# anyboby/Constrained-Model-Based-Policy-Optimization

Measured on AMD Instinct MI355X. Metric: imagined env-steps/sec (ensemble rollout) + CPO update ms, higher is better.
Workload: dtype f32; 1 GPU; AntSafe-v2 imagined rollout: E=7 x (37->512->512->60) swish ensemble, 5 elites, 3+3 critics 128x128, tanh policy 128x128, B=100000 branches/GPU, maxroll 35 (34 steps), fixed-horizon mode, reset->sample*->finish_all_paths->get(); rollout_mode=schedule, branches_per_gpu=100000, branches_total=100000, horizon=34, task=AntSafe-v2

## Files before the change

constrained-model-based-policy-optimization_amd/csrc/ens_h3.hip:

```cpp
#include "common.h"
#include "ens_mlp_internal.h"
#include "f16_split.h"

#include <stdlib.h>

#include <type_traits>

namespace {

constexpr int kThreadsH = 512;
constexpr int kWavesH = 8;
constexpr int HIDH = 512;

template <int RT>
struct Geo {
  static constexpr int ROWS = 32 * RT;
  static constexpr int NTC = 8 / RT;
  static constexpr int CK = 32 * NTC;
  static constexpr int NCH = HIDH / CK;
  static constexpr int SLC = CK / 16;
  static constexpr int CSTR = CK + 8;
  static constexpr int TPR = kThreadsH / ROWS;
  static constexpr int KPT = 64 / TPR;
  static constexpr int DA = RT == 4 ? 2 : 4;
  static constexpr int CBUF_BYTES = 2 * ROWS * CSTR * 2;
  static constexpr bool W0_LDS = RT == 4;
};

constexpr int PBUF_BYTES = kWavesH * 2 * 16 * 64 * 4;
constexpr int SWS = 65;
constexpr int STG_BYTES = 32 * SWS * 4;
__host__ __device__ constexpr int ximg_bytes(int S0, int RT) { return 2 * 32 * RT * (16 * S0 + 8) * 2; }
__host__ __device__ constexpr int w0buf_bytes(int S0, int RT) { return RT == 4 ? 2 * S0 * 2 * 1024 : 0; }
__host__ __device__ constexpr int off_const(int S0, int RT) {
  const int cb = RT == 4 ? Geo<4>::CBUF_BYTES : (RT == 2 ? Geo<2>::CBUF_BYTES : Geo<1>::CBUF_BYTES);
  const int a = 2 * cb + ximg_bytes(S0, RT) + 2 * w0buf_bytes(S0, RT), b = 2 * PBUF_BYTES + 2 * STG_BYTES;
  return ((a > b ? a : b) + 15) / 16 * 16;
}
constexpr int CONST_FLOATS = 2 * HIDH + 2 * 128 + 6 * 128 + 2 * 64;
// ... 33 lines not shown
  __shared__ float red[3][kThreadsH];
  red[0][tid] = wmax; red[1][tid] = l1; red[2][tid] = bmax;
  __syncthreads();
  for (int st = kThreadsH / 2; st > 0; st >>= 1) {
    if (tid < st)
      for (int q = 0; q < 3; ++q) red[q][tid] = fmaxf(red[q][tid], red[q][tid + st]);
    __syncthreads();
  }
  if (tid == 0) {
    float *o = stats + (size_t)e * NSTAT + 4 * l;
    o[0] = pow2_lift(red[0][0]); o[1] = red[1][0]; o[2] = red[2][0]; o[3] = red[0][0];
  }
}

__global__ void h3_pack_kernel(const float *src, size_t src_stride, int kg, int src_tiles, f16x8 *dst, size_t dst_stride,
                               int n_tiles, int slabs, int members, const float *stats, int layer, int perm) {
  const long idx = (long)blockIdx.x * blockDim.x + threadIdx.x;
  const long per = (long)n_tiles * slabs * 64;
  if (idx >= per * members) return;
  const int e = (int)(idx / per);
  const int rem = (int)(idx - (long)e * per);
  const int lane = rem & 63, s = (rem >> 6) % slabs, tile = (rem >> 6) / slabs;
  const int r = lane & 31, h = lane >> 5;
  const float scale = stats[(size_t)e * NSTAT + 4 * layer];
  const float *sp = src + (size_t)e * src_stride;
  f16x8 p1, p2;
#pragma unroll
  for (int j = 0; j < 8; ++j) {
    int k = 16 * s + 8 * h + j;
    if (perm) {
      const int i = 8 * (s & 1) + j;
      k = 32 * (s >> 1) + (i & 3) + 8 * (i >> 2) + 4 * h;
    }
    float v = 0.0f;
    if (tile < src_tiles && (k >> 3) < kg) v = sp[(((size_t)tile * kg + (k >> 3)) * 64 + ((k >> 2) & 1) * 32 + r) * 4 + (k & 3)];
    _Float16 q1, q2;
    split_h(v * scale, q1, q2);
    p1[j] = q1; p2[j] = q2;
  }
  f16x8 *d = dst + (size_t)e * dst_stride + ((size_t)tile * slabs + s) * 2 * 64 + lane;
  d[0] = p1; d[64] = p2;
}

template <int I, int N, class F>
__device__ __forceinline__ void static_for(F &&f) {
  if constexpr (I < N) {
    f(std::integral_constant<int, I>{});
    static_for<I + 1, N>(f);
  }
}

#ifdef H3_FULL_BARRIERS
#define H3_BARRIER() __syncthreads()
#else
#define H3_BARRIER() asm volatile("s_waitcnt lgkmcnt(0)\n\ts_barrier" ::: "memory")
#endif

#ifndef H3_EPI_FUSE
#define H3_EPI_FUSE 1
#endif
#ifndef IN_SCALE_RCP
#define IN_SCALE_RCP 1
#endif
#ifndef H3_PEEL_LAST
#define H3_PEEL_LAST 1
#endif
#ifndef H3_STORE8
#define H3_STORE8 1
#endif
#ifndef H3_TAIL_RING
#define H3_TAIL_RING 0
#endif

struct H3Args {
  MlpKernelArgs m;
  const f16x8 *w0, *w1, *w2;
  size_t w0_stride, w1_stride, w2_stride;
  const float *stats;
  int item0;
};

template <int S0, int OTP, int RT>
__global__ __launch_bounds__(kThreadsH, 2) void ens_h3_kernel(const H3Args a) {
  using G = Geo<RT>;
  constexpr int ROWSH = G::ROWS, NTC = G::NTC, CK = G::CK, NCH = G::NCH, SLC = G::SLC, CSTR = G::CSTR, TPR = G::TPR,
                KPT = G::KPT, DA = G::DA, CBUF_BYTES = G::CBUF_BYTES;
  constexpr int XSTR = 16 * S0 + 8;
  constexpr int NPASS = OTP / 2;
  constexpr int NUNIT = RT * NPASS;
  constexpr int O_PAD = 32 * OTP;
  constexpr int W0P = NTC * S0 * 2;
  const MlpKernelArgs &p = a.m;
  extern __shared__ f32x4 smem4[];
  char *smem = reinterpret_cast<char *>(smem4);
  _Float16 *cbuf = reinterpret_cast<_Float16 *>(smem);
  _Float16 *ximg = reinterpret_cast<_Float16 *>(smem + 2 * CBUF_BYTES);
  f16x8 *w0buf = reinterpret_cast<f16x8 *>(smem + 2 * CBUF_BYTES + ximg_bytes(S0, RT));
  f32x4 *pbuf = reinterpret_cast<f32x4 *>(smem);
  float *stg = reinterpret_cast<float *>(smem + 2 * PBUF_BYTES);
  float *cst = reinterpret_cast<float *>(smem + off_const(S0, RT));
  float *bias0 = cst, *bias1 = cst + HIDH, *hc_a = cst + 2 * HIDH, *hc_c = hc_a + 128;
// ... 154 lines not shown
      const f16x8 *wa = G::W0_LDS ? w0buf + ((size_t)(cc & 1) * W0P + (size_t)l0_tn * S0 * 2 + 2 * s) * 64 + lane
                                  : w0e + (((size_t)(cc < NCH ? cc : NCH - 1) * NTC + l0_tn) * S0 * 2 + 2 * s) * 64 + lane;
      o.a1 = wa[0]; o.a2 = wa[64];
      o.b1 = *reinterpret_cast<const f16x8 *>(xb0 + 16 * s);
      o.b2 = *reinterpret_cast<const f16x8 *>(xb0 + (size_t)ROWSH * XSTR + 16 * s);
    };
    auto l0_store = [&](const Epi4 &s, int cc, int q) {
      _Float16 *c1 = cbuf + (size_t)(cc & 1) * (CBUF_BYTES / 2) + (size_t)(32 * l0_bt + r) * CSTR + 32 * l0_tn + 4 * hh + 8 * q;
      *reinterpret_cast<uint2 *>(c1) = make_uint2(s.q1[0], s.q1[1]);
      *reinterpret_cast<uint2 *>(c1 + (size_t)ROWSH * CSTR) = make_uint2(s.q2[0], s.q2[1]);
    };
    auto l0_bias = [&](int cc, int q) {
      return *reinterpret_cast<const f32x4 *>(bias0 + cc * CK + 32 * l0_tn + 8 * q + 4 * hh);
    };

    f32x16 acc[2][RT];
#pragma unroll
    for (int t = 0; t < 2; ++t)
#pragma unroll
      for (int bt = 0; bt < RT; ++bt)
#pragma unroll
        for (int i = 0; i < 16; ++i) acc[t][bt][i] = 0.0f;
    const f16x8 *w1a = a.w1 + (size_t)e * a.w1_stride + (size_t)(2 * wave) * 32 * 128 + lane;
    f16x8 A[DA][2][2];
    f16x8 Bt[3][2];
    auto load_a = [&](f16x8 (&x)[2][2], int s) {
#pragma unroll
      for (int t = 0; t < 2; ++t) {
        const f16x8 *q = w1a + ((size_t)t * 32 + s) * 128;
        x[t][0] = q[0]; x[t][1] = q[64];
      }
    };
    auto read_bt = [&](f16x8 (&x)[2], const _Float16 *img, int bt, int sl) {
      const _Float16 *q = img + (size_t)(32 * bt + r) * CSTR + 16 * sl + 8 * hh;
      x[0] = *reinterpret_cast<const f16x8 *>(q);
      x[1] = *reinterpret_cast<const f16x8 *>(q + (size_t)ROWSH * CSTR);
    };
#pragma unroll
    for (int s = 0; s < DA - 1; ++s) load_a(A[s], s);
    {
      f32x16 d;
#pragma unroll
      for (int i = 0; i < 16; ++i) d[i] = 0.0f;
#pragma unroll
      for (int s = 0; s < S0; ++s) {
        L0Ops o;
        l0_read(o, 0, s);
        mm3(d, o.a1, o.a2, o.b1, o.b2);
      }
#pragma unroll
      for (int q = 0; q < 4; ++q) {
        Epi4 es;
        const f32x4 bv = l0_bias(0, q);
        epi_all<false, true, H3_EPI_FUSE>(es, d, q, inv0_l, bv, t1_l);
        l0_store(es, 0, q);
      }
    }
    H3_BARRIER();
    H3_STAMP(2);

    auto step = [&](auto LASTC, const int c) {
      constexpr bool LAST = decltype(LASTC)::value;
      f16x8 wst;
      const bool stage_w0 = c + 2 < NCH;
      const int cw = stage_w0 ? c + 2 : NCH - 1;
      const _Float16 *img = cbuf + (size_t)(c & 1) * (CBUF_BYTES / 2);
      f32x16 d;
#pragma unroll
      for (int i = 0; i < 16; ++i) d[i] = 0.0f;
      L0Ops l0;
      Epi4 es;
      f32x4 bv = {0.0f, 0.0f, 0.0f, 0.0f};
      read_bt(Bt[0], img, 0, 0);
      read_bt(Bt[1], img, 1 % RT, 1 / RT);
      if constexpr (!LAST) l0_read(l0, c + 1, 0);
#pragma unroll
      for (int slot = 0; slot < 8; ++slot) {
        if (!LAST && slot >= 4) bv = l0_bias(c + 1, slot - 4);
        if constexpr (G::W0_LDS && !LAST) {
          if (slot == 4) wst = w0e[((size_t)cw * W0P + wave) * 64 + lane];
          if (slot == 5 && W0P > kWavesH) {
            if (stage_w0) w0buf[((size_t)(c & 1) * W0P + wave) * 64 + lane] = wst;
            wst = w0e[((size_t)cw * W0P + (wave + kWavesH < W0P ? wave + kWavesH : wave)) * 64 + lane];
          }
        }
#pragma unroll
        for (int i = 0; i < 12; ++i) {
          const int pos = 2 * slot + i / 6;
          const int sl = pos / RT, bt = pos % RT;
          const int t = (i / 3) % 2, term = i % 3;
          if (i % 6 == 0) {
#ifndef H3_DIAG_NOA
            if (bt == 0) {
              const int sn = c * SLC + sl + DA - 1;
              load_a(A[(sl + DA - 1) % DA], sn < 32 ? sn : 31);
            }
#endif
#ifndef H3_DIAG_NOBT
            if (pos + 2 < 16) read_bt(Bt[(pos + 2) % 3], img, (pos + 2) % RT, (pos + 2) / RT);
#endif
            if (i == 0) __builtin_amdgcn_sched_barrier(0);
          }
          f16x8(&Ac)[2][2] = A[sl % DA];
          f32x16 &ac = acc[t][bt];
          const f16x8 &b1 = Bt[pos % 3][0], &b2 = Bt[pos % 3][1];
          if (term == 0) ac = __builtin_amdgcn_mfma_f32_32x32x16_f16(Ac[t][1], b1, ac, 0, 0, 0);
          else if (term == 1) ac = __builtin_amdgcn_mfma_f32_32x32x16_f16(Ac[t][0], b2, ac, 0, 0, 0);
          else ac = __builtin_amdgcn_mfma_f32_32x32x16_f16(Ac[t][0], b1, ac, 0, 0, 0);
#ifndef H3_DIAG_NOL0
          if (!LAST && slot < S0 && i == 5) {
            mm3(d, l0.a1, l0.a2, l0.b1, l0.b2);
            if (slot + 1 < S0) l0_read(l0, c + 1, slot + 1);
          }
#endif
#ifdef H3_DIAG_NOEPI_LOOP
          if (false) {
#else
          if (!LAST && slot >= 4) {
#endif
            const int q = slot - 4;
            if (i == 0) epi_stage<0, true, true, H3_EPI_FUSE>(es, d, q, inv0_l, bv, t1_l);
            if (i == 1) epi_stage<1, true, true, H3_EPI_FUSE>(es, d, q, inv0_l, bv, t1_l);
            if (i == 2) epi_stage<2, true, true, H3_EPI_FUSE>(es, d, q, inv0_l, bv, t1_l);
            if (i == 3) epi_stage<3, true, true, H3_EPI_FUSE>(es, d, q, inv0_l, bv, t1_l);
            if (i == 4) epi_stage<4, true, true, H3_EPI_FUSE>(es, d, q, inv0_l, bv, t1_l);
            if (i == 5) epi_stage<5, true, true, H3_EPI_FUSE>(es, d, q, inv0_l, bv, t1_l);
            if (i == 6) epi_stage<6, true, true, H3_EPI_FUSE>(es, d, q, inv0_l, bv, t1_l);
            if (i == 7) epi_stage<7, true, true, H3_EPI_FUSE>(es, d, q, inv0_l, bv, t1_l);
            if (i == 8) epi_stage<8, true, true, H3_EPI_FUSE>(es, d, q, inv0_l, bv, t1_l);
            if (i == 9) epi_stage<9, true, true, H3_EPI_FUSE>(es, d, q, inv0_l, bv, t1_l);
            if (i == 10) l0_store(es, c + 1, q);
          }
          __builtin_amdgcn_sched_barrier(0);
        }
      }
      H3_STAMP(4);
      if constexpr (G::W0_LDS && !LAST) {
        if (stage_w0) {
          const int j = W0P > kWavesH ? wave + kWavesH : wave;
          if (j < W0P) w0buf[((size_t)(c & 1) * W0P + j) * 64 + lane] = wst;
        }
      }
      H3_BARRIER();
      H3_STAMP(5);
    };
#if H3_PEEL_LAST
#pragma unroll 1
    for (int c = 0; c < NCH - 1; ++c) step(std::false_type{}, c);
    step(std::true_type{}, NCH - 1);
#else
#pragma unroll 1
    for (int c = 0; c < NCH; ++c) step(std::false_type{}, c);
#endif

    fetch_x(tid);
    fetch_bias(item + gridDim.x, tid);
    H3_STAMP(6);
#ifdef H3_DIAG_NOTAIL
    {
      float keep = 0.0f;
#pragma unroll
      for (int t = 0; t < 2; ++t)
#pragma unroll
        for (int bt = 0; bt < RT; ++bt)
#pragma unroll
          for (int i = 0; i < 16; ++i) keep += acc[t][bt][i];
      if (keep == 123.456f) p.out0[0] = keep;
    }
    H3_BARRIER();
    continue;
#endif

    const f16x8 *w2w = a.w2 + (size_t)e * a.w2_stride + lane + (size_t)(4 * wave) * 128;
    auto reduce_unit = [&](int u) {
      const int rt = u / NPASS, pass = u % NPASS;
      const int tt = wave >> 2, q = wave & 3;
      const f32x4 *pp = pbuf + ((size_t)(u & 1) * 64 + (size_t)tt * 4 + q) * 64 + lane;
      f32x4 v = pp[0];
#pragma unroll
      for (int wv = 1; wv < kWavesH; ++wv) v += pp[(size_t)wv * 8 * 64];
      const int nl = 32 * tt + 8 * q + 4 * hh, n = 64 * pass + nl;
      const f32x4 ha = *reinterpret_cast<const f32x4 *>(hc_a + n), hc = *reinterpret_cast<const f32x4 *>(hc_c + n);
      const float inv2_l = r_inv2[32 * rt + r];
      float *sg = stg + (size_t)(u & 1) * 32 * SWS + r * SWS + nl;
#pragma unroll
      for (int s = 0; s < 4; ++s) {
        float y = ha[s] * (v[s] * inv2_l) + hc[s];
        if (n + s >= out) y = __expf(y);
// ... 19 lines not shown
        return;
      }
      const int n = 64 * pass + lane;
#pragma unroll
      for (int j = 0; j < 4; ++j) {
        const int rl = wave + kWavesH * j;
        const int rr = rowidx[32 * rt + rl];
        const float y = stg[(size_t)(u & 1) * 32 * SWS + rl * SWS + lane];
        if (rr >= 0 && n < 2 * out) {
          const size_t obase = ((size_t)e * p.ld_rows + rr) * out;
          if (n < out) p.out0[obase + n] = y;
          else p.out1[obase + (n - out)] = y;
        }
      }
    };
    if constexpr (NPASS == 1 && !H3_TAIL_RING) {
      f16x8 w2r[4][2][2];
      static_for<0, 4>([&](auto SI) {
        constexpr int S = decltype(SI)::value;
#pragma unroll
        for (int tt = 0; tt < 2; ++tt) {
          const f16x8 *q = w2w + ((size_t)tt * 32 + S) * 128;
          w2r[S][tt][0] = q[0]; w2r[S][tt][1] = q[64];
        }
      });
      u32x4 bfu[2][4][2];
      auto stA = [&](auto RTI) {
        constexpr int rt = decltype(RTI)::value;
        const float inv1_l = r_inv1[32 * rt + r] * kLog2e;
        const float t2_l = H3_EPI_FUSE ? pow2_rcp(r_t2[32 * rt + r]) * kLog2e : r_t2[32 * rt + r] * kLn2;
        static_for<0, 8>([&](auto QD) {
          constexpr int quad = decltype(QD)::value, S = quad >> 1, jq = quad & 1, q = 2 * (S & 1) + jq;
          const f32x4 bv = *reinterpret_cast<const f32x4 *>(bias1 + 64 * wave + 32 * (S >> 1) + 8 * q + 4 * hh);
          Epi4 es;
#ifdef H3_DIAG_TAIL_NOA
          es.q1[0] = __float_as_uint(acc[S >> 1][rt][4 * q] + bv[0]) & 0x3fff3fffu; es.q1[1] = __float_as_uint(acc[S >> 1][rt][4 * q + 1] + inv1_l) & 0x3fff3fffu;
          es.q2[0] = __float_as_uint(acc[S >> 1][rt][4 * q + 2] + t2_l) & 0x3fff3fffu; es.q2[1] = __float_as_uint(acc[S >> 1][rt][4 * q + 3]) & 0x3fff3fffu;
#else
          epi_all<false, true, H3_EPI_FUSE>(es, acc[S >> 1][rt], q, inv1_l, bv, t2_l);
#endif
          bfu[rt & 1][S][0][2 * jq] = es.q1[0]; bfu[rt & 1][S][0][2 * jq + 1] = es.q1[1];
          bfu[rt & 1][S][1][2 * jq] = es.q2[0]; bfu[rt & 1][S][1][2 * jq + 1] = es.q2[1];
        });
      };
      auto stB = [&](auto RTI) {
        constexpr int rt = decltype(RTI)::value;
        f32x16 o[2];
#pragma unroll
        for (int tt = 0; tt < 2; ++tt)
#pragma unroll
          for (int i = 0; i < 16; ++i) o[tt][i] = 0.0f;
        static_for<0, 4>([&](auto SI) {
          constexpr int S = decltype(SI)::value;
          const f16x8 b1 = __builtin_bit_cast(f16x8, bfu[rt & 1][S][0]), b2 = __builtin_bit_cast(f16x8, bfu[rt & 1][S][1]);
#ifdef H3_DIAG_TAIL_NOB
#pragma unroll
          for (int tt = 0; tt < 2; ++tt) { o[tt][S] += (float)b1[tt] + (float)w2r[S][tt][0][0]; o[tt][S + 4] += (float)b2[tt] + (float)w2r[S][tt][1][1]; }
#else
#pragma unroll
          for (int tt = 0; tt < 2; ++tt) mm3(o[tt], w2r[S][tt][0], w2r[S][tt][1], b1, b2);
#endif
        });
        f32x4 *pw = pbuf + ((size_t)(rt & 1) * 64 + (size_t)wave * 8) * 64 + lane;
#pragma unroll
        for (int tt = 0; tt < 2; ++tt)
#pragma unroll
          for (int q = 0; q < 4; ++q) {
            const f32x4 v = {o[tt][4 * q], o[tt][4 * q + 1], o[tt][4 * q + 2], o[tt][4 * q + 3]};
            pw[(size_t)(tt * 4 + q) * 64] = v;
          }
      };
      stA(std::integral_constant<int, 0>{});
      static_for<0, RT + 2>([&](auto KI) {
        constexpr int k = decltype(KI)::value;
        auto matrix_side = [&]() {
#ifndef H3_DIAG_TAIL_NOD
          if constexpr (k >= 2 && k - 2 < RT) store_unit(k - 2);
#endif
#ifndef H3_DIAG_TAIL_NOC
          if constexpr (k >= 1 && k - 1 < RT) reduce_unit(k - 1);
#endif
          if constexpr (k < RT) stB(std::integral_constant<int, (k < RT ? k : 0)>{});
        };
        auto valu_side = [&]() {
          if constexpr (k + 1 < RT) stA(std::integral_constant<int, (k + 1 < RT ? k + 1 : 0)>{});
        };
#ifdef H3_TAIL_STAGGER
        if (k == 0 || wave < 4) { matrix_side(); valu_side(); }
        else { valu_side(); matrix_side(); }
#else
        matrix_side(); valu_side();
#endif
        H3_STAMP(7);
        if constexpr (k + 1 < RT + 2) H3_BARRIER();
        H3_STAMP(8);
      });
    } else {
#pragma unroll
    for (int rt = 0; rt < RT; ++rt) {
      f16x8 wf[2][2][2];
      auto load_w2 = [&](f16x8 (&x)[2][2], int pass, int S) {
#pragma unroll
        for (int tt = 0; tt < 2; ++tt) {
          const f16x8 *q = w2w + ((size_t)(2 * pass + tt) * 32 + S) * 128;
          x[tt][0] = q[0]; x[tt][1] = q[64];
        }
      };
      load_w2(wf[0], 0, 0);
      f16x8 bf[4][2];
      {
        u32x4 bfu[4][2];
        const float inv1_l = r_inv1[32 * rt + r] * kLog2e;
        const float t2_l = H3_EPI_FUSE ? pow2_rcp(r_t2[32 * rt + r]) * kLog2e : r_t2[32 * rt + r] * kLn2;
#pragma unroll
        for (int S = 0; S < 4; ++S)
#pragma unroll
          for (int jq = 0; jq < 2; ++jq) {
            const int q = 2 * (S & 1) + jq;
            const f32x4 bv = *reinterpret_cast<const f32x4 *>(bias1 + 64 * wave + 32 * (S >> 1) + 8 * q + 4 * hh);
            Epi4 es;
            epi_all<false, true, H3_EPI_FUSE>(es, acc[S >> 1][rt], q, inv1_l, bv, t2_l);
            bfu[S][0][2 * jq] = es.q1[0]; bfu[S][0][2 * jq + 1] = es.q1[1];
            bfu[S][1][2 * jq] = es.q2[0]; bfu[S][1][2 * jq + 1] = es.q2[1];
          }
#pragma unroll
        for (int S = 0; S < 4; ++S)
#pragma unroll
          for (int pc = 0; pc < 2; ++pc) bf[S][pc] = __builtin_bit_cast(f16x8, bfu[S][pc]);
      }
#pragma unroll
      for (int pass = 0; pass < NPASS; ++pass) {
        const int u = rt * NPASS + pass;
        f32x16 o[2];
#pragma unroll
        for (int tt = 0; tt < 2; ++tt)
#pragma unroll
          for (int i = 0; i < 16; ++i) o[tt][i] = 0.0f;
#pragma unroll
        for (int S = 0; S < 4; ++S) {
          const int nS = (S + 1) & 3, npass = (S == 3) ? pass + 1 : pass;
          if (S < 3 || pass + 1 < NPASS) load_w2(wf[(S & 1) ^ 1], npass, nS);
#pragma unroll
          for (int tt = 0; tt < 2; ++tt) mm3(o[tt], wf[S & 1][tt][0], wf[S & 1][tt][1], bf[S][0], bf[S][1]);
        }
        f32x4 *pw = pbuf + ((size_t)(u & 1) * 64 + (size_t)wave * 8) * 64 + lane;
#pragma unroll
        for (int tt = 0; tt < 2; ++tt)
#pragma unroll
          for (int q = 0; q < 4; ++q) {
            const f32x4 v = {o[tt][4 * q], o[tt][4 * q + 1], o[tt][4 * q + 2], o[tt][4 * q + 3]};
            pw[(size_t)(tt * 4 + q) * 64] = v;
          }
        H3_STAMP(7);
        H3_BARRIER();
        H3_STAMP(8);
        if (u > 0) store_unit(u - 1);
        reduce_unit(u);
        H3_STAMP(9);
      }
    }
    H3_BARRIER();
    store_unit(NUNIT - 1);
    }
    H3_STAMP(10);
    H3_BARRIER();
    H3_STAMP(11);
  }
#ifdef CMBPO_STAMPS
  if (p.stamps && threadIdx.x == 0) {
    for (int k = 0; k < 12; ++k) p.stamps[(size_t)blockIdx.x * 16 + k] = t_acc[k];
    p.stamps[(size_t)blockIdx.x * 16 + 12] = __builtin_amdgcn_s_memrealtime() - t_rt0;
  }
#endif
}

}

static int ensure_h3(cmbpo_mlp *m, hipStream_t s) {
  const int H = m->hidden, E = m->ensemble;
  const int S0 = m->h3_s0, OTP = m->h3_otp;
  const int slabs[3] = {S0, H / 16, H / 16};
  const int tiles[3] = {H / 32, H / 32, OTP};
  if (m->d_h3 == nullptr) {
    size_t off = 0;
    for (int l = 0; l < 3; ++l) {
      m->h3_stride[l] = (size_t)tiles[l] * slabs[l] * 2 * 64;
      m->h3_off[l] = off;
      off += m->h3_stride[l] * E;
    }
    m->h3_stats_off = off;
    const size_t bytes = off * 16 + (size_t)E * NSTAT * sizeof(float);
    if (hipMalloc(&m->d_h3, bytes) != hipSuccess) {
      (void)hipGetLastError();
      m->d_h3 = nullptr;
      cmbpo_set_error("ens_h3: hipMalloc of the f16 weight images failed");
      return CMBPO_ENOMEM;
    }
    m->h3_version = ~0ul;
  }
  if (m->h3_version == m->pack_version) return CMBPO_OK;
  float *stats = reinterpret_cast<float *>(reinterpret_cast<char *>(m->d_h3) + m->h3_stats_off * 16);
  hipLaunchKernelGGL(h3_stats_kernel, dim3(E, 3), dim3(kThreadsH), 0, s, m->d_blob, m->off_wp0, m->off_wp1, m->off_wp2,
                     m->off_b0, m->off_b1, m->off_b2, m->in_pad / 8, m->o_tiles, H, stats);
  const size_t src_off[3] = {m->off_wp0, m->off_wp1, m->off_wp2};
  const int kg[3] = {m->in_pad / 8, H / 8, H / 8};
  const int src_tiles[3] = {H / 32, H / 32, m->o_tiles};
  for (int l = 0; l < 3; ++l) {
    const size_t src_stride = (size_t)src_tiles[l] * kg[l] * 256;
    const long total = (long)tiles[l] * slabs[l] * 64 * E;
    hipLaunchKernelGGL(h3_pack_kernel, dim3((unsigned)((total + 255) / 256)), dim3(256), 0, s, m->d_blob + src_off[l], src_stride,
                       kg[l], src_tiles[l], reinterpret_cast<f16x8 *>(m->d_h3) + m->h3_off[l], m->h3_stride[l], tiles[l], slabs[l],
                       E, stats, l, l == 2 ? 1 : 0);
  }
  CMBPO_HIP_CHECK(hipGetLastError());
  m->h3_version = m->pack_version;
  return CMBPO_OK;
}

void cmbpo_internal_f16_stats(const cmbpo_mlp *m, float *stats, hipStream_t s) {
  hipLaunchKernelGGL(h3_stats_kernel, dim3(m->ensemble, 3), dim3(kThreadsH), 0, s, m->d_blob, m->off_wp0, m->off_wp1, m->off_wp2,
                     m->off_b0, m->off_b1, m->off_b2, m->in_pad / 8, m->o_tiles, m->hidden, stats);
}
void cmbpo_internal_f16_pack(const cmbpo_mlp *m, int layer, void *dst, size_t dst_stride, int n_tiles, int slabs, int perm,
                             const float *stats, hipStream_t s) {
  const int H = m->hidden;
  const size_t src_off[3] = {m->off_wp0, m->off_wp1, m->off_wp2};
  const int kg[3] = {m->in_pad / 8, H / 8, H / 8};
// ... 95 lines not shown
```

constrained-model-based-policy-optimization_amd/csrc/f16_split.h:

```cpp
#pragma once
#include "common.h"

typedef _Float16 f16x8 __attribute__((ext_vector_type(8)));
typedef _Float16 f16x4 __attribute__((ext_vector_type(4)));
typedef unsigned u32x4 __attribute__((ext_vector_type(4)));

constexpr int NSTAT = 12;

__device__ __forceinline__ float swishf(float x) { return x * __builtin_amdgcn_rcpf(1.0f + __expf(-x)); }

__host__ __device__ __forceinline__ float pow2_lift(float v) {
  union { float f; unsigned u; } c;
  c.f = v;
  const int ex = (int)((c.u >> 23) & 255u);
  if (ex == 0 || ex == 255) return 1.0f;
  int k = 13 - (ex - 127);
  k = k < -100 ? -100 : (k > 100 ? 100 : k);
  c.u = (unsigned)(k + 127) << 23;
  return c.f;
}

#ifndef POW2_RCP
#define POW2_RCP 1
#endif
// ... 6 lines not shown
#else
  return 1.0f / x;
#endif
}

__device__ __forceinline__ void split_h(float a, _Float16 &p1, _Float16 &p2) {
  p1 = (_Float16)a;
  p2 = (_Float16)(a - (float)p1);
}

__device__ __forceinline__ void mm3(f32x16 &acc, const f16x8 &a1, const f16x8 &a2, const f16x8 &b1, const f16x8 &b2) {
  acc = __builtin_amdgcn_mfma_f32_32x32x16_f16(a2, b1, acc, 0, 0, 0);
  acc = __builtin_amdgcn_mfma_f32_32x32x16_f16(a1, b2, acc, 0, 0, 0);
  acc = __builtin_amdgcn_mfma_f32_32x32x16_f16(a1, b1, acc, 0, 0, 0);
}

template <bool HAZ>
__device__ __forceinline__ void split2(float x0, float x1, float t, unsigned &q1, unsigned &q2) {
  unsigned a, b;
  asm("v_fma_mixlo_f16 %0, %1, %2, 0" : "=&v"(a) : "v"(x0), "v"(t));
  if constexpr (HAZ) asm("v_fma_mixhi_f16 %0, %1, %2, 0\n\ts_nop 1" : "+v"(a) : "v"(x1), "v"(t));
  else asm("v_fma_mixhi_f16 %0, %1, %2, 0" : "+v"(a) : "v"(x1), "v"(t));
  asm("v_fma_mixlo_f16 %0, %1, %2, -%3 op_sel:[0,0,0] op_sel_hi:[0,0,1]" : "=&v"(b) : "v"(x0), "v"(t), "v"(a));
  if constexpr (HAZ) asm("v_fma_mixhi_f16 %0, %1, %2, -%3 op_sel:[0,0,1] op_sel_hi:[0,0,1]\n\ts_nop 1" : "+v"(b) : "v"(x1), "v"(t), "v"(a));
  else asm("v_fma_mixhi_f16 %0, %1, %2, -%3 op_sel:[0,0,1] op_sel_hi:[0,0,1]" : "+v"(b) : "v"(x1), "v"(t), "v"(a));
  q1 = a;
  q2 = b;
}

struct Epi4 {
  float z[4], e[4];
  unsigned q1[2], q2[2];
};
constexpr float kLog2e = 1.4426950408889634f, kLn2 = 0.6931471805599453f;
template <int K, bool PIN, bool PRE = false, bool FUSE = false>
__device__ __forceinline__ void epi_stage(Epi4 &s, const f32x16 &d, int q, float inv, const f32x4 &bv, float tn) {
  if constexpr (PRE && K == 1) {
  } else if constexpr (PRE && (K == 2 || K == 3)) {
    constexpr int o = 2 * (K - 2);
    s.e[o] = __builtin_amdgcn_exp2f(-s.z[o]); s.e[o + 1] = __builtin_amdgcn_exp2f(-s.z[o + 1]);
    if (PIN) asm volatile("" : "+v"(s.e[o]), "+v"(s.e[o + 1]));
  } else if constexpr (K == 0) {
#pragma unroll
    for (int i = 0; i < 4; ++i) s.z[i] = __builtin_fmaf(d[4 * q + i], inv, bv[i]);
    if (PIN) asm volatile("" : "+v"(s.z[0]), "+v"(s.z[1]), "+v"(s.z[2]), "+v"(s.z[3]));
  } else if constexpr (K == 1) {
#pragma unroll
    for (int i = 0; i < 4; ++i) s.e[i] = s.z[i] * -1.4426950408889634f;
    if (PIN) asm volatile("" : "+v"(s.e[0]), "+v"(s.e[1]), "+v"(s.e[2]), "+v"(s.e[3]));
  } else if constexpr (K == 2 || K == 3) {
    constexpr int o = 2 * (K - 2);
// ... 43 lines not shown
    if (PIN) asm volatile("" : "+v"(s.q1[0]), "+v"(s.q1[1]));
  } else if constexpr (K == 9) {
    const float m0 = FUSE ? s.e[0] : tn, m1 = FUSE ? s.e[1] : tn, m2 = FUSE ? s.e[2] : tn, m3 = FUSE ? s.e[3] : tn;
    asm("v_fma_mixlo_f16 %0, %1, %2, -%3 op_sel:[0,0,0] op_sel_hi:[0,0,1]" : "=&v"(s.q2[0]) : "v"(s.z[0]), "v"(m0), "v"(s.q1[0]));
    asm("v_fma_mixlo_f16 %0, %1, %2, -%3 op_sel:[0,0,0] op_sel_hi:[0,0,1]" : "=&v"(s.q2[1]) : "v"(s.z[2]), "v"(m2), "v"(s.q1[1]));
    if constexpr (PIN) {
      asm("v_fma_mixhi_f16 %0, %1, %2, -%3 op_sel:[0,0,1] op_sel_hi:[0,0,1]" : "+v"(s.q2[0]) : "v"(s.z[1]), "v"(m1), "v"(s.q1[0]));
      asm("v_fma_mixhi_f16 %0, %1, %2, -%3 op_sel:[0,0,1] op_sel_hi:[0,0,1]" : "+v"(s.q2[1]) : "v"(s.z[3]), "v"(m3), "v"(s.q1[1]));
    } else {
      asm("v_fma_mixhi_f16 %0, %1, %2, -%3 op_sel:[0,0,1] op_sel_hi:[0,0,1]\n\ts_nop 1" : "+v"(s.q2[0]) : "v"(s.z[1]), "v"(m1), "v"(s.q1[0]));
      asm("v_fma_mixhi_f16 %0, %1, %2, -%3 op_sel:[0,0,1] op_sel_hi:[0,0,1]\n\ts_nop 1" : "+v"(s.q2[1]) : "v"(s.z[3]), "v"(m3), "v"(s.q1[1]));
    }
    if (PIN) asm volatile("" : "+v"(s.q2[0]), "+v"(s.q2[1]));
  }
}
template <bool PIN, bool PRE = false, bool FUSE = false>
__device__ __forceinline__ void epi_all(Epi4 &s, const f32x16 &d, int q, float inv, const f32x4 &bv, float tn) {
  epi_stage<0, PIN, PRE, FUSE>(s, d, q, inv, bv, tn); epi_stage<1, PIN, PRE, FUSE>(s, d, q, inv, bv, tn);
  epi_stage<2, PIN, PRE, FUSE>(s, d, q, inv, bv, tn); epi_stage<3, PIN, PRE, FUSE>(s, d, q, inv, bv, tn);
  epi_stage<4, PIN, PRE, FUSE>(s, d, q, inv, bv, tn); epi_stage<5, PIN, PRE, FUSE>(s, d, q, inv, bv, tn);
  epi_stage<6, PIN, PRE, FUSE>(s, d, q, inv, bv, tn); epi_stage<7, PIN, PRE, FUSE>(s, d, q, inv, bv, tn);
  epi_stage<8, PIN, PRE, FUSE>(s, d, q, inv, bv, tn); epi_stage<9, PIN, PRE, FUSE>(s, d, q, inv, bv, tn);
}


struct cmbpo_mlp;
void cmbpo_internal_f16_stats(const cmbpo_mlp *m, float *stats, hipStream_t s);
void cmbpo_internal_f16_pack(const cmbpo_mlp *m, int layer, void *dst, size_t dst_stride, int n_tiles, int slabs, int perm,
                             const float *stats, hipStream_t s);
```

Measured before the change: 69.27 million imagined env-steps/s.

## Switch hidden and output layers to 16x16x32 MFMA tiles with new weight packing

Rewrites the layer-1 main loop and the layer-2 tail of the fused ensemble MLP kernel so they use 16x16x32 f16 MFMAs with f32x4 accumulators instead of 32x32x16 with f32x16. The pack kernel gains modes that lay out the weights as 16-row tiles, and the A-fragment prefetch ring is now indexed by a half-slab phase, with the chunk loop unrolled by phase. The aim is better MFMA scheduling granularity and interleaving of loads and epilogue work, at the cost of more MFMA instructions and more fragment bookkeeping. Diagnostic macros and the peel and tail-ring options are removed.

```diff
diff --git a/constrained-model-based-policy-optimization_amd/csrc/ens_h3.hip b/constrained-model-based-policy-optimization_amd/csrc/ens_h3.hip
--- a/constrained-model-based-policy-optimization_amd/csrc/ens_h3.hip
+++ b/constrained-model-based-policy-optimization_amd/csrc/ens_h3.hip
@@ -18,11 +18,12 @@
   static constexpr int NTC = 8 / RT;
   static constexpr int CK = 32 * NTC;
   static constexpr int NCH = HIDH / CK;
-  static constexpr int SLC = CK / 16;
+  static constexpr int SLC = CK / 32;
   static constexpr int CSTR = CK + 8;
   static constexpr int TPR = kThreadsH / ROWS;
   static constexpr int KPT = 64 / TPR;
-  static constexpr int DA = RT == 4 ? 2 : 4;
+  static constexpr int DH = RT == 4 ? 2 : 4;
+  static constexpr int NPH = (2 * SLC) % DH == 0 ? 1 : DH;
   static constexpr int CBUF_BYTES = 2 * ROWS * CSTR * 2;
   static constexpr bool W0_LDS = RT == 4;
 };
@@ -86,26 +87,30 @@
 }
 
 __global__ void h3_pack_kernel(const float *src, size_t src_stride, int kg, int src_tiles, f16x8 *dst, size_t dst_stride,
-                               int n_tiles, int slabs, int members, const float *stats, int layer, int perm) {
+                               int n_tiles, int slabs, int members, const float *stats, int layer, int mode) {
   const long idx = (long)blockIdx.x * blockDim.x + threadIdx.x;
   const long per = (long)n_tiles * slabs * 64;
   if (idx >= per * members) return;
   const int e = (int)(idx / per);
   const int rem = (int)(idx - (long)e * per);
   const int lane = rem & 63, s = (rem >> 6) % slabs, tile = (rem >> 6) / slabs;
-  const int r = lane & 31, h = lane >> 5;
+  const bool m16 = mode >= 2;
+  const int n = m16 ? 16 * tile + (lane & 15) : 32 * tile + (lane & 31);
+  const int r = n & 31, g = m16 ? lane >> 4 : lane >> 5;
   const float scale = stats[(size_t)e * NSTAT + 4 * layer];
   const float *sp = src + (size_t)e * src_stride;
   f16x8 p1, p2;
 #pragma unroll
   for (int j = 0; j < 8; ++j) {
-    int k = 16 * s + 8 * h + j;
-    if (perm) {
+    int k;
+    if (mode == 0) k = 16 * s + 8 * g + j;
+    else if (mode == 1) {
       const int i = 8 * (s & 1) + j;
-      k = 32 * (s >> 1) + (i & 3) + 8 * (i >> 2) + 4 * h;
-    }
+      k = 32 * (s >> 1) + (i & 3) + 8 * (i >> 2) + 4 * g;
+    } else if (mode == 2) k = 32 * s + 8 * ((g & 1) * 2 + (g >> 1)) + j;
+    else k = 32 * s + 16 * (j >> 2) + 4 * g + (j & 3);
     float v = 0.0f;
-    if (tile < src_tiles && (k >> 3) < kg) v = sp[(((size_t)tile * kg + (k >> 3)) * 64 + ((k >> 2) & 1) * 32 + r) * 4 + (k & 3)];
+    if ((n >> 5) < src_tiles && (k >> 3) < kg) v = sp[(((size_t)(n >> 5) * kg + (k >> 3)) * 64 + ((k >> 2) & 1) * 32 + r) * 4 + (k & 3)];
     _Float16 q1, q2;
     split_h(v * scale, q1, q2);
     p1[j] = q1; p2[j] = q2;
@@ -134,14 +139,8 @@
 #ifndef IN_SCALE_RCP
 #define IN_SCALE_RCP 1
 #endif
-#ifndef H3_PEEL_LAST
-#define H3_PEEL_LAST 1
-#endif
 #ifndef H3_STORE8
 #define H3_STORE8 1
-#endif
-#ifndef H3_TAIL_RING
-#define H3_TAIL_RING 0
 #endif
 
 struct H3Args {
@@ -156,7 +155,7 @@
 __global__ __launch_bounds__(kThreadsH, 2) void ens_h3_kernel(const H3Args a) {
   using G = Geo<RT>;
   constexpr int ROWSH = G::ROWS, NTC = G::NTC, CK = G::CK, NCH = G::NCH, SLC = G::SLC, CSTR = G::CSTR, TPR = G::TPR,
-                KPT = G::KPT, DA = G::DA, CBUF_BYTES = G::CBUF_BYTES;
+                KPT = G::KPT, DH = G::DH, NPH = G::NPH, CBUF_BYTES = G::CBUF_BYTES;
   constexpr int XSTR = 16 * S0 + 8;
   constexpr int NPASS = OTP / 2;
   constexpr int NUNIT = RT * NPASS;
@@ -341,30 +340,35 @@
       return *reinterpret_cast<const f32x4 *>(bias0 + cc * CK + 32 * l0_tn + 8 * q + 4 * hh);
     };
 
-    f32x16 acc[2][RT];
-#pragma unroll
-    for (int t = 0; t < 2; ++t)
-#pragma unroll
-      for (int bt = 0; bt < RT; ++bt)
-#pragma unroll
-        for (int i = 0; i < 16; ++i) acc[t][bt][i] = 0.0f;
-    const f16x8 *w1a = a.w1 + (size_t)e * a.w1_stride + (size_t)(2 * wave) * 32 * 128 + lane;
-    f16x8 A[DA][2][2];
-    f16x8 Bt[3][2];
-    auto load_a = [&](f16x8 (&x)[2][2], int s) {
+    constexpr int VT = 2 * RT;
+    const int c16 = lane & 15, g4 = lane >> 4;
+    const int sig = c16 < 4 ? 2 * c16 : (c16 < 12 ? 2 * c16 - 7 : 2 * c16 - 16);
+    const int pik = 8 * (2 * (g4 & 1) + (g4 >> 1));
+    f32x4 acc[4][VT];
+#pragma unroll
+    for (int u = 0; u < 4; ++u)
+#pragma unroll
+      for (int v = 0; v < VT; ++v)
+#pragma unroll
+        for (int i = 0; i < 4; ++i) acc[u][v][i] = 0.0f;
+    const f16x8 *w1a = a.w1 + (size_t)e * a.w1_stride + (size_t)(4 * wave) * 16 * 128 + lane;
+    f16x8 A[DH][2][2];
+    f16x8 Bt[2][2];
+    auto load_h = [&](f16x8 (&x)[2][2], int h) {
+      h = h < 31 ? h : 31;
 #pragma unroll
       for (int t = 0; t < 2; ++t) {
-        const f16x8 *q = w1a + ((size_t)t * 32 + s) * 128;
+        const f16x8 *q = w1a + ((size_t)(2 * (h & 1) + t) * 16 + (h >> 1)) * 128;
         x[t][0] = q[0]; x[t][1] = q[64];
       }
     };
-    auto read_bt = [&](f16x8 (&x)[2], const _Float16 *img, int bt, int sl) {
-      const _Float16 *q = img + (size_t)(32 * bt + r) * CSTR + 16 * sl + 8 * hh;
+    auto read_b = [&](f16x8 (&x)[2], const _Float16 *img, int v, int sl) {
+      const _Float16 *q = img + (size_t)(16 * v + sig) * CSTR + 32 * sl + pik;
       x[0] = *reinterpret_cast<const f16x8 *>(q);
       x[1] = *reinterpret_cast<const f16x8 *>(q + (size_t)ROWSH * CSTR);
     };
 #pragma unroll
-    for (int s = 0; s < DA - 1; ++s) load_a(A[s], s);
+    for (int h = 0; h < DH; ++h) load_h(A[h], h);
     {
       f32x16 d;
 #pragma unroll
@@ -386,8 +390,9 @@
     H3_BARRIER();
     H3_STAMP(2);
 
-    auto step = [&](auto LASTC, const int c) {
+    auto step = [&](auto LASTC, const int c, auto PHC) {
       constexpr bool LAST = decltype(LASTC)::value;
+      constexpr int PH = decltype(PHC)::value;
       f16x8 wst;
       const bool stage_w0 = c + 2 < NCH;
       const int cw = stage_w0 ? c + 2 : NCH - 1;
@@ -398,8 +403,7 @@
       L0Ops l0;
       Epi4 es;
       f32x4 bv = {0.0f, 0.0f, 0.0f, 0.0f};
-      read_bt(Bt[0], img, 0, 0);
-      read_bt(Bt[1], img, 1 % RT, 1 / RT);
+      read_b(Bt[0], img, 0, 0);
       if constexpr (!LAST) l0_read(l0, c + 1, 0);
 #pragma unroll
       for (int slot = 0; slot < 8; ++slot) {
@@ -412,51 +416,40 @@
           }
         }
 #pragma unroll
-        for (int i = 0; i < 12; ++i) {
-          const int pos = 2 * slot + i / 6;
-          const int sl = pos / RT, bt = pos % RT;
-          const int t = (i / 3) % 2, term = i % 3;
-          if (i % 6 == 0) {
-#ifndef H3_DIAG_NOA
-            if (bt == 0) {
-              const int sn = c * SLC + sl + DA - 1;
-              load_a(A[(sl + DA - 1) % DA], sn < 32 ? sn : 31);
-            }
-#endif
-#ifndef H3_DIAG_NOBT
-            if (pos + 2 < 16) read_bt(Bt[(pos + 2) % 3], img, (pos + 2) % RT, (pos + 2) / RT);
-#endif
+        for (int i = 0; i < 24; ++i) {
+          const int pos = 2 * slot + i / 12;
+          const int sl = pos / VT, v = pos % VT;
+          const int u = (i % 12) / 3, term = i % 3;
+          const int hl = 2 * sl + (u >> 1);
+          f16x8(&Ah)[2][2] = A[(PH * 2 * SLC + hl) % DH];
+          if (i % 12 == 0) {
+            if (pos + 1 < 16) read_b(Bt[(pos + 1) & 1], img, (pos + 1) % VT, (pos + 1) / VT);
             if (i == 0) __builtin_amdgcn_sched_barrier(0);
           }
-          f16x8(&Ac)[2][2] = A[sl % DA];
-          f32x16 &ac = acc[t][bt];
-          const f16x8 &b1 = Bt[pos % 3][0], &b2 = Bt[pos % 3][1];
-          if (term == 0) ac = __builtin_amdgcn_mfma_f32_32x32x16_f16(Ac[t][1], b1, ac, 0, 0, 0);
-          else if (term == 1) ac = __builtin_amdgcn_mfma_f32_32x32x16_f16(Ac[t][0], b2, ac, 0, 0, 0);
-          else ac = __builtin_amdgcn_mfma_f32_32x32x16_f16(Ac[t][0], b1, ac, 0, 0, 0);
-#ifndef H3_DIAG_NOL0
-          if (!LAST && slot < S0 && i == 5) {
+          f32x4 &ac = acc[u][v];
+          const f16x8 &b1 = Bt[pos & 1][0], &b2 = Bt[pos & 1][1];
+          if (term == 0) ac = __builtin_amdgcn_mfma_f32_16x16x32_f16(Ah[u & 1][1], b1, ac, 0, 0, 0);
+          else if (term == 1) ac = __builtin_amdgcn_mfma_f32_16x16x32_f16(Ah[u & 1][0], b2, ac, 0, 0, 0);
+          else ac = __builtin_amdgcn_mfma_f32_16x16x32_f16(Ah[u & 1][0], b1, ac, 0, 0, 0);
+          if (v == VT - 1 && (i % 12 == 5 || i % 12 == 11) && !(LAST && hl + DH >= 2 * SLC))
+            load_h(Ah, c * 2 * SLC + hl + DH);
+          if (!LAST && slot < S0 && i == 11) {
             mm3(d, l0.a1, l0.a2, l0.b1, l0.b2);
             if (slot + 1 < S0) l0_read(l0, c + 1, slot + 1);
           }
-#endif
-#ifdef H3_DIAG_NOEPI_LOOP
-          if (false) {
-#else
-          if (!LAST && slot >= 4) {
-#endif
-            const int q = slot - 4;
-            if (i == 0) epi_stage<0, true, true, H3_EPI_FUSE>(es, d, q, inv0_l, bv, t1_l);
-            if (i == 1) epi_stage<1, true, true, H3_EPI_FUSE>(es, d, q, inv0_l, bv, t1_l);
-            if (i == 2) epi_stage<2, true, true, H3_EPI_FUSE>(es, d, q, inv0_l, bv, t1_l);
-            if (i == 3) epi_stage<3, true, true, H3_EPI_FUSE>(es, d, q, inv0_l, bv, t1_l);
-            if (i == 4) epi_stage<4, true, true, H3_EPI_FUSE>(es, d, q, inv0_l, bv, t1_l);
-            if (i == 5) epi_stage<5, true, true, H3_EPI_FUSE>(es, d, q, inv0_l, bv, t1_l);
-            if (i == 6) epi_stage<6, true, true, H3_EPI_FUSE>(es, d, q, inv0_l, bv, t1_l);
-            if (i == 7) epi_stage<7, true, true, H3_EPI_FUSE>(es, d, q, inv0_l, bv, t1_l);
-            if (i == 8) epi_stage<8, true, true, H3_EPI_FUSE>(es, d, q, inv0_l, bv, t1_l);
-            if (i == 9) epi_stage<9, true, true, H3_EPI_FUSE>(es, d, q, inv0_l, bv, t1_l);
-            if (i == 10) l0_store(es, c + 1, q);
+          if (!LAST && slot >= 4 && i % 2 == 0) {
+            const int q = slot - 4, k = i / 2;
+            if (k == 0) epi_stage<0, true, true, H3_EPI_FUSE>(es, d, q, inv0_l, bv, t1_l);
+            if (k == 1) epi_stage<1, true, true, H3_EPI_FUSE>(es, d, q, inv0_l, bv, t1_l);
+            if (k == 2) epi_stage<2, true, true, H3_EPI_FUSE>(es, d, q, inv0_l, bv, t1_l);
+            if (k == 3) epi_stage<3, true, true, H3_EPI_FUSE>(es, d, q, inv0_l, bv, t1_l);
+            if (k == 4) epi_stage<4, true, true, H3_EPI_FUSE>(es, d, q, inv0_l, bv, t1_l);
+            if (k == 5) epi_stage<5, true, true, H3_EPI_FUSE>(es, d, q, inv0_l, bv, t1_l);
+            if (k == 6) epi_stage<6, true, true, H3_EPI_FUSE>(es, d, q, inv0_l, bv, t1_l);
+            if (k == 7) epi_stage<7, true, true, H3_EPI_FUSE>(es, d, q, inv0_l, bv, t1_l);
+            if (k == 8) epi_stage<8, true, true, H3_EPI_FUSE>(es, d, q, inv0_l, bv, t1_l);
+            if (k == 9) epi_stage<9, true, true, H3_EPI_FUSE>(es, d, q, inv0_l, bv, t1_l);
+            if (k == 10) l0_store(es, c + 1, q);
           }
           __builtin_amdgcn_sched_barrier(0);
         }
@@ -471,14 +464,14 @@
       H3_BARRIER();
       H3_STAMP(5);
     };
-#if H3_PEEL_LAST
+    {
+      constexpr int NREG = NCH - 1, NFULL = NREG / NPH * NPH;
 #pragma unroll 1
-    for (int c = 0; c < NCH - 1; ++c) step(std::false_type{}, c);
-    step(std::true_type{}, NCH - 1);
-#else
-#pragma unroll 1
-    for (int c = 0; c < NCH; ++c) step(std::false_type{}, c);
-#endif
+      for (int c0 = 0; c0 < NFULL; c0 += NPH)
+        static_for<0, NPH>([&](auto P) { step(std::false_type{}, c0 + decltype(P)::value, P); });
+      static_for<0, NREG - NFULL>([&](auto P) { step(std::false_type{}, NFULL + decltype(P)::value, P); });
+      step(std::true_type{}, NREG, std::integral_constant<int, NREG % NPH>{});
+    }
 
     fetch_x(tid);
     fetch_bias(item + gridDim.x, tid);
@@ -487,18 +480,18 @@
     {
       float keep = 0.0f;
 #pragma unroll
-      for (int t = 0; t < 2; ++t)
-#pragma unroll
-        for (int bt = 0; bt < RT; ++bt)
-#pragma unroll
-          for (int i = 0; i < 16; ++i) keep += acc[t][bt][i];
+      for (int u = 0; u < 4; ++u)
+#pragma unroll
+        for (int v = 0; v < VT; ++v)
+#pragma unroll
+          for (int i = 0; i < 4; ++i) keep += acc[u][v][i];
       if (keep == 123.456f) p.out0[0] = keep;
     }
     H3_BARRIER();
     continue;
 #endif
 
-    const f16x8 *w2w = a.w2 + (size_t)e * a.w2_stride + lane + (size_t)(4 * wave) * 128;
+    const f16x8 *w2w = a.w2 + (size_t)e * a.w2_stride + lane;
     auto reduce_unit = [&](int u) {
       const int rt = u / NPASS, pass = u % NPASS;
       const int tt = wave >> 2, q = wave & 3;
@@ -548,153 +541,118 @@
         }
       }
     };
-    if constexpr (NPASS == 1 && !H3_TAIL_RING) {
-      f16x8 w2r[4][2][2];
-      static_for<0, 4>([&](auto SI) {
-        constexpr int S = decltype(SI)::value;
-#pragma unroll
-        for (int tt = 0; tt < 2; ++tt) {
-          const f16x8 *q = w2w + ((size_t)tt * 32 + S) * 128;
-          w2r[S][tt][0] = q[0]; w2r[S][tt][1] = q[64];
-        }
-      });
-      u32x4 bfu[2][4][2];
-      auto stA = [&](auto RTI) {
-        constexpr int rt = decltype(RTI)::value;
-        const float inv1_l = r_inv1[32 * rt + r] * kLog2e;
-        const float t2_l = H3_EPI_FUSE ? pow2_rcp(r_t2[32 * rt + r]) * kLog2e : r_t2[32 * rt + r] * kLn2;
-        static_for<0, 8>([&](auto QD) {
-          constexpr int quad = decltype(QD)::value, S = quad >> 1, jq = quad & 1, q = 2 * (S & 1) + jq;
-          const f32x4 bv = *reinterpret_cast<const f32x4 *>(bias1 + 64 * wave + 32 * (S >> 1) + 8 * q + 4 * hh);
+    auto h2_frag = [&](u32x4 (&bfu)[2][2][2], auto RTI) {
+      constexpr int rt = decltype(RTI)::value;
+#pragma unroll
+      for (int vv = 0; vv < 2; ++vv) {
+        const int row = 32 * rt + 16 * vv + sig;
+        const float inv1_l = r_inv1[row] * kLog2e;
+        const float t2_l = H3_EPI_FUSE ? pow2_rcp(r_t2[row]) * kLog2e : r_t2[row] * kLn2;
+#pragma unroll
+        for (int u = 0; u < 4; ++u) {
+          const f32x4 bv = *reinterpret_cast<const f32x4 *>(bias1 + 64 * wave + 16 * u + 4 * g4);
           Epi4 es;
-#ifdef H3_DIAG_TAIL_NOA
-          es.q1[0] = __float_as_uint(acc[S >> 1][rt][4 * q] + bv[0]) & 0x3fff3fffu; es.q1[1] = __float_as_uint(acc[S >> 1][rt][4 * q + 1] + inv1_l) & 0x3fff3fffu;
-          es.q2[0] = __float_as_uint(acc[S >> 1][rt][4 * q + 2] + t2_l) & 0x3fff3fffu; es.q2[1] = __float_as_uint(acc[S >> 1][rt][4 * q + 3]) & 0x3fff3fffu;
-#else
-          epi_all<false, true, H3_EPI_FUSE>(es, acc[S >> 1][rt], q, inv1_l, bv, t2_l);
-#endif
-          bfu[rt & 1][S][0][2 * jq] = es.q1[0]; bfu[rt & 1][S][0][2 * jq + 1] = es.q1[1];
-          bfu[rt & 1][S][1][2 * jq] = es.q2[0]; bfu[rt & 1][S][1][2 * jq + 1] = es.q2[1];
-        });
-      };
+          epi_all<false, true, H3_EPI_FUSE>(es, acc[u][2 * rt + vv], 0, inv1_l, bv, t2_l);
+          bfu[vv][u >> 1][0][2 * (u & 1)] = es.q1[0]; bfu[vv][u >> 1][0][2 * (u & 1) + 1] = es.q1[1];
+          bfu[vv][u >> 1][1][2 * (u & 1)] = es.q2[0]; bfu[vv][u >> 1][1][2 * (u & 1) + 1] = es.q2[1];
+        }
+      }
+    };
+    auto out_mm = [&](f32x4 (&o)[2][2], const f16x8 (&w)[2][2], const u32x4 (&bfu)[2][2][2], int ks) {
+#pragma unroll
+      for (int vv = 0; vv < 2; ++vv) {
+        const f16x8 b1 = __builtin_bit_cast(f16x8, bfu[vv][ks][0]), b2 = __builtin_bit_cast(f16x8, bfu[vv][ks][1]);
+#pragma unroll
+        for (int aa = 0; aa < 2; ++aa) mm3(o[aa][vv], w[aa][0], w[aa][1], b1, b2);
+      }
+    };
+    auto put_partials = [&](const f32x4 (&o)[2][2][2], int u) {
+      f32x4 *pw = pbuf + ((size_t)(u & 1) * 64 + (size_t)wave * 8) * 64;
+#pragma unroll
+      for (int tt = 0; tt < 2; ++tt)
+#pragma unroll
+        for (int aa = 0; aa < 2; ++aa)
+#pragma unroll
+          for (int vv = 0; vv < 2; ++vv)
+            pw[(size_t)(tt * 4 + 2 * aa + (g4 >> 1)) * 64 + 16 * vv + sig + 32 * (g4 & 1)] = o[tt][aa][vv];
+    };
+    auto zero_o = [&](f32x4 (&o)[2][2][2]) {
+#pragma unroll
+      for (int tt = 0; tt < 2; ++tt)
+#pragma unroll
+        for (int aa = 0; aa < 2; ++aa)
+#pragma unroll
+          for (int vv = 0; vv < 2; ++vv)
+#pragma unroll
+            for (int i = 0; i < 4; ++i) o[tt][aa][vv][i] = 0.0f;
+    };
+    if constexpr (NPASS == 1) {
+      f16x8 w2r[2][2][2][2];
+#pragma unroll
+      for (int ks = 0; ks < 2; ++ks)
+#pragma unroll
+        for (int ot = 0; ot < 4; ++ot) {
+          const f16x8 *q = w2w + ((size_t)ot * 16 + 2 * wave + ks) * 128;
+          w2r[ks][ot >> 1][ot & 1][0] = q[0]; w2r[ks][ot >> 1][ot & 1][1] = q[64];
+        }
+      u32x4 bfu[2][2][2][2];
+      auto stA = [&](auto RTI) { h2_frag(bfu[decltype(RTI)::value & 1], RTI); };
       auto stB = [&](auto RTI) {
         constexpr int rt = decltype(RTI)::value;
-        f32x16 o[2];
-#pragma unroll
-        for (int tt = 0; tt < 2; ++tt)
-#pragma unroll
-          for (int i = 0; i < 16; ++i) o[tt][i] = 0.0f;
-        static_for<0, 4>([&](auto SI) {
-          constexpr int S = decltype(SI)::value;
-          const f16x8 b1 = __builtin_bit_cast(f16x8, bfu[rt & 1][S][0]), b2 = __builtin_bit_cast(f16x8, bfu[rt & 1][S][1]);
-#ifdef H3_DIAG_TAIL_NOB
-#pragma unroll
-          for (int tt = 0; tt < 2; ++tt) { o[tt][S] += (float)b1[tt] + (float)w2r[S][tt][0][0]; o[tt][S + 4] += (float)b2[tt] + (float)w2r[S][tt][1][1]; }
-#else
-#pragma unroll
-          for (int tt = 0; tt < 2; ++tt) mm3(o[tt], w2r[S][tt][0], w2r[S][tt][1], b1, b2);
-#endif
-        });
-        f32x4 *pw = pbuf + ((size_t)(rt & 1) * 64 + (size_t)wave * 8) * 64 + lane;
-#pragma unroll
-        for (int tt = 0; tt < 2; ++tt)
-#pragma unroll
-          for (int q = 0; q < 4; ++q) {
-            const f32x4 v = {o[tt][4 * q], o[tt][4 * q + 1], o[tt][4 * q + 2], o[tt][4 * q + 3]};
-            pw[(size_t)(tt * 4 + q) * 64] = v;
-          }
+        f32x4 o[2][2][2];
+        zero_o(o);
+#pragma unroll
+        for (int ks = 0; ks < 2; ++ks)
+#pragma unroll
+          for (int tt = 0; tt < 2; ++tt) out_mm(o[tt], w2r[ks][tt], bfu[rt & 1], ks);
+        put_partials(o, rt);
       };
       stA(std::integral_constant<int, 0>{});
       static_for<0, RT + 2>([&](auto KI) {
         constexpr int k = decltype(KI)::value;
-        auto matrix_side = [&]() {
-#ifndef H3_DIAG_TAIL_NOD
-          if constexpr (k >= 2 && k - 2 < RT) store_unit(k - 2);
-#endif
-#ifndef H3_DIAG_TAIL_NOC
-          if constexpr (k >= 1 && k - 1 < RT) reduce_unit(k - 1);
-#endif
-          if constexpr (k < RT) stB(std::integral_constant<int, (k < RT ? k : 0)>{});
-        };
-        auto valu_side = [&]() {
-          if constexpr (k + 1 < RT) stA(std::integral_constant<int, (k + 1 < RT ? k + 1 : 0)>{});
-        };
-#ifdef H3_TAIL_STAGGER
-        if (k == 0 || wave < 4) { matrix_side(); valu_side(); }
-        else { valu_side(); matrix_side(); }
-#else
-        matrix_side(); valu_side();
-#endif
+        if constexpr (k >= 2 && k - 2 < RT) store_unit(k - 2);
+        if constexpr (k >= 1 && k - 1 < RT) reduce_unit(k - 1);
+        if constexpr (k < RT) stB(std::integral_constant<int, (k < RT ? k : 0)>{});
+        if constexpr (k + 1 < RT) stA(std::integral_constant<int, (k + 1 < RT ? k + 1 : 0)>{});
         H3_STAMP(7);
         if constexpr (k + 1 < RT + 2) H3_BARRIER();
         H3_STAMP(8);
       });
     } else {
-#pragma unroll
-    for (int rt = 0; rt < RT; ++rt) {
-      f16x8 wf[2][2][2];
-      auto load_w2 = [&](f16x8 (&x)[2][2], int pass, int S) {
-#pragma unroll
-        for (int tt = 0; tt < 2; ++tt) {
-          const f16x8 *q = w2w + ((size_t)(2 * pass + tt) * 32 + S) * 128;
-          x[tt][0] = q[0]; x[tt][1] = q[64];
-        }
-      };
-      load_w2(wf[0], 0, 0);
-      f16x8 bf[4][2];
-      {
-        u32x4 bfu[4][2];
-        const float inv1_l = r_inv1[32 * rt + r] * kLog2e;
-        const float t2_l = H3_EPI_FUSE ? pow2_rcp(r_t2[32 * rt + r]) * kLog2e : r_t2[32 * rt + r] * kLn2;
-#pragma unroll
-        for (int S = 0; S < 4; ++S)
-#pragma unroll
-          for (int jq = 0; jq < 2; ++jq) {
-            const int q = 2 * (S & 1) + jq;
-            const f32x4 bv = *reinterpret_cast<const f32x4 *>(bias1 + 64 * wave + 32 * (S >> 1) + 8 * q + 4 * hh);
-            Epi4 es;
-            epi_all<false, true, H3_EPI_FUSE>(es, acc[S >> 1][rt], q, inv1_l, bv, t2_l);
-            bfu[S][0][2 * jq] = es.q1[0]; bfu[S][0][2 * jq + 1] = es.q1[1];
-            bfu[S][1][2 * jq] = es.q2[0]; bfu[S][1][2 * jq + 1] = es.q2[1];
+      static_for<0, RT>([&](auto RTI) {
+        constexpr int rt = decltype(RTI)::value;
+        f16x8 wf[2][2][2];
+        auto load_w2 = [&](f16x8 (&x)[2][2], int pass, int st) {
+#pragma unroll
+          for (int aa = 0; aa < 2; ++aa) {
+            const f16x8 *q = w2w + ((size_t)(4 * pass + 2 * (st & 1) + aa) * 16 + 2 * wave + (st >> 1)) * 128;
+            x[aa][0] = q[0]; x[aa][1] = q[64];
           }
-#pragma unroll
-        for (int S = 0; S < 4; ++S)
-#pragma unroll
-          for (int pc = 0; pc < 2; ++pc) bf[S][pc] = __builtin_bit_cast(f16x8, bfu[S][pc]);
-      }
-#pragma unroll
-      for (int pass = 0; pass < NPASS; ++pass) {
-        const int u = rt * NPASS + pass;
-        f32x16 o[2];
-#pragma unroll
-        for (int tt = 0; tt < 2; ++tt)
-#pragma unroll
-          for (int i = 0; i < 16; ++i) o[tt][i] = 0.0f;
-#pragma unroll
-        for (int S = 0; S < 4; ++S) {
-          const int nS = (S + 1) & 3, npass = (S == 3) ? pass + 1 : pass;
-          if (S < 3 || pass + 1 < NPASS) load_w2(wf[(S & 1) ^ 1], npass, nS);
-#pragma unroll
-          for (int tt = 0; tt < 2; ++tt) mm3(o[tt], wf[S & 1][tt][0], wf[S & 1][tt][1], bf[S][0], bf[S][1]);
-        }
-        f32x4 *pw = pbuf + ((size_t)(u & 1) * 64 + (size_t)wave * 8) * 64 + lane;
-#pragma unroll
-        for (int tt = 0; tt < 2; ++tt)
-#pragma unroll
-          for (int q = 0; q < 4; ++q) {
-            const f32x4 v = {o[tt][4 * q], o[tt][4 * q + 1], o[tt][4 * q + 2], o[tt][4 * q + 3]};
-            pw[(size_t)(tt * 4 + q) * 64] = v;
+        };
+        load_w2(wf[0], 0, 0);
+        u32x4 bfu[2][2][2];
+        h2_frag(bfu, RTI);
+#pragma unroll
+        for (int pass = 0; pass < NPASS; ++pass) {
+          const int u = rt * NPASS + pass;
+          f32x4 o[2][2][2];
+          zero_o(o);
+#pragma unroll
+          for (int st = 0; st < 4; ++st) {
+            if (st < 3 || pass + 1 < NPASS) load_w2(wf[(st & 1) ^ 1], st == 3 ? pass + 1 : pass, (st + 1) & 3);
+            out_mm(o[st & 1], wf[st & 1], bfu, st >> 1);
           }
-        H3_STAMP(7);
-        H3_BARRIER();
-        H3_STAMP(8);
-        if (u > 0) store_unit(u - 1);
-        reduce_unit(u);
-        H3_STAMP(9);
-      }
-    }
-    H3_BARRIER();
-    store_unit(NUNIT - 1);
+          put_partials(o, u);
+          H3_STAMP(7);
+          H3_BARRIER();
+          H3_STAMP(8);
+          if (u > 0) store_unit(u - 1);
+          reduce_unit(u);
+          H3_STAMP(9);
+        }
+      });
+      H3_BARRIER();
+      store_unit(NUNIT - 1);
     }
     H3_STAMP(10);
     H3_BARRIER();
@@ -713,8 +671,8 @@
 static int ensure_h3(cmbpo_mlp *m, hipStream_t s) {
   const int H = m->hidden, E = m->ensemble;
   const int S0 = m->h3_s0, OTP = m->h3_otp;
-  const int slabs[3] = {S0, H / 16, H / 16};
-  const int tiles[3] = {H / 32, H / 32, OTP};
+  const int slabs[3] = {S0, H / 32, H / 32};
+  const int tiles[3] = {H / 32, H / 16, 2 * OTP};
   if (m->d_h3 == nullptr) {
     size_t off = 0;
     for (int l = 0; l < 3; ++l) {
@@ -744,7 +702,7 @@
     const long total = (long)tiles[l] * slabs[l] * 64 * E;
     hipLaunchKernelGGL(h3_pack_kernel, dim3((unsigned)((total + 255) / 256)), dim3(256), 0, s, m->d_blob + src_off[l], src_stride,
                        kg[l], src_tiles[l], reinterpret_cast<f16x8 *>(m->d_h3) + m->h3_off[l], m->h3_stride[l], tiles[l], slabs[l],
-                       E, stats, l, l == 2 ? 1 : 0);
+                       E, stats, l, l == 0 ? 0 : l + 1);
   }
   CMBPO_HIP_CHECK(hipGetLastError());
   m->h3_version = m->pack_version;
diff --git a/constrained-model-based-policy-optimization_amd/csrc/f16_split.h b/constrained-model-based-policy-optimization_amd/csrc/f16_split.h
--- a/constrained-model-based-policy-optimization_amd/csrc/f16_split.h
+++ b/constrained-model-based-policy-optimization_amd/csrc/f16_split.h
@@ -44,6 +44,11 @@
   acc = __builtin_amdgcn_mfma_f32_32x32x16_f16(a1, b2, acc, 0, 0, 0);
   acc = __builtin_amdgcn_mfma_f32_32x32x16_f16(a1, b1, acc, 0, 0, 0);
 }
+__device__ __forceinline__ void mm3(f32x4 &acc, const f16x8 &a1, const f16x8 &a2, const f16x8 &b1, const f16x8 &b2) {
+  acc = __builtin_amdgcn_mfma_f32_16x16x32_f16(a2, b1, acc, 0, 0, 0);
+  acc = __builtin_amdgcn_mfma_f32_16x16x32_f16(a1, b2, acc, 0, 0, 0);
+  acc = __builtin_amdgcn_mfma_f32_16x16x32_f16(a1, b1, acc, 0, 0, 0);
+}
 
 template <bool HAZ>
 __device__ __forceinline__ void split2(float x0, float x1, float t, unsigned &q1, unsigned &q2) {
@@ -63,8 +68,8 @@
   unsigned q1[2], q2[2];
 };
 constexpr float kLog2e = 1.4426950408889634f, kLn2 = 0.6931471805599453f;
-template <int K, bool PIN, bool PRE = false, bool FUSE = false>
-__device__ __forceinline__ void epi_stage(Epi4 &s, const f32x16 &d, int q, float inv, const f32x4 &bv, float tn) {
+template <int K, bool PIN, bool PRE = false, bool FUSE = false, class D>
+__device__ __forceinline__ void epi_stage(Epi4 &s, const D &d, int q, float inv, const f32x4 &bv, float tn) {
   if constexpr (PRE && K == 1) {
   } else if constexpr (PRE && (K == 2 || K == 3)) {
     constexpr int o = 2 * (K - 2);
@@ -138,8 +143,8 @@
     if (PIN) asm volatile("" : "+v"(s.q2[0]), "+v"(s.q2[1]));
   }
 }
-template <bool PIN, bool PRE = false, bool FUSE = false>
-__device__ __forceinline__ void epi_all(Epi4 &s, const f32x16 &d, int q, float inv, const f32x4 &bv, float tn) {
+template <bool PIN, bool PRE = false, bool FUSE = false, class D>
+__device__ __forceinline__ void epi_all(Epi4 &s, const D &d, int q, float inv, const f32x4 &bv, float tn) {
   epi_stage<0, PIN, PRE, FUSE>(s, d, q, inv, bv, tn); epi_stage<1, PIN, PRE, FUSE>(s, d, q, inv, bv, tn);
   epi_stage<2, PIN, PRE, FUSE>(s, d, q, inv, bv, tn); epi_stage<3, PIN, PRE, FUSE>(s, d, q, inv, bv, tn);
   epi_stage<4, PIN, PRE, FUSE>(s, d, q, inv, bv, tn); epi_stage<5, PIN, PRE, FUSE>(s, d, q, inv, bv, tn);
```

Result: faster. 72.95 million imagined env-steps/s, median of 6 (+5.3%).
